# soedinglab/spacedust

Hardware: AMD Instinct MI355X
Metric: clustersearch throughput (genome-pairs/s; SW GCUPS alongside) (higher is better)
Workload: dtype int16

## Files before the change

spacedust_amd/csrc/hip/sd_sw.hip:

```cpp
#include "sd_common.h"
#include <unistd.h>


#include <algorithm>
#include <cmath>
#include <cstring>
#include <memory>
#include <omp.h>
#include <numeric>

#include "../host/sd_host.h"
#include "sd_sw_pk.h"

namespace {

using sdpk::SwTask;

template <int RT>
__global__ void __launch_bounds__(64)
sw_score_kernel(const SwTask *__restrict__ tasks, uint32_t nTasks, const uint8_t *__restrict__ qRes,
                const int8_t *__restrict__ qBias, const uint8_t *__restrict__ tRes, const int8_t *__restrict__ mat,
                int go, int ge, int32_t *__restrict__ out, uint2 *__restrict__ boundary,
                const uint32_t *__restrict__ order ,
                const int8_t *__restrict__ qProf ) {
// ... 613 lines not shown
            x = jj - x;
            ok = ok && x >= 0 && x < width_d;
            bool same = false;
            if (ok) {
                const int byte = dirs[(size_t) 16 * ii + (x >> 1)];
                const int code = (x & 1) ? (byte >> 4) : (byte & 15);
                ok = (code & 12) == 0;
                same = sq[ii] == st[jj];
            }
            const uint32_t okMask = (uint32_t) (__ballot(ok) >> sh);
            const uint32_t sameMask = (uint32_t) (__ballot(same) >> sh);
            const int run = okMask == 0xFFFFFFFFu ? 32 : __builtin_ctz(~okMask);
            const uint32_t runMask = run == 32 ? 0xFFFFFFFFu : ((1u << run) - 1u);
            if (l < run) o[-1 - l] = 'M';
            ids += __builtin_popcount(sameMask & runMask);
            i -= run;
            j -= run;
            o -= run;
            len += run;
        }
        if (going && (i > 0 || j > 0)) {
            if (i < 0 || j < 0) bad = true;
            int x = i - band;
            x = x > 0 ? x : 0;
            x = j - x;
            if (x < 0 || x >= width_d) bad = true;
            if (!bad) {
                const int byte = dirs[(size_t) 16 * i + (x >> 1)];
                const int code = (x & 1) ? (byte >> 4) : (byte & 15);
                int dcode;
                const int dE = (code & 1) ? 3 : 2, dF = (code & 2) ? 5 : 4;
                if (state == 0) dcode = dE;
                else if (state == 1) dcode = dF;
                else dcode = (code & 4) ? dE : ((code & 8) ? dF : 1);
                char c;
                switch (dcode) {
                    case 1: ids += (sq[i] == st[j]); --i; --j; state = 2; c = 'M'; break;
                    case 2: --i; state = 0; c = 'I'; break;
                    case 3: --i; state = 2; c = 'I'; break;
                    case 4: --j; state = 1; c = 'D'; break;
                    default: --j; state = 2; c = 'D'; break;
                }
                --o;
                if (l == 0) *o = c;
                len++;
            }
        }
        going = going && !bad && (i > 0 || j > 0);
    }
    if (!have || !reached || l != 0) return;
    if (bad || i != 0 || j != 0) {
        res[2 * id] = -1;
        return;
    }
    ids += (sq[0] == st[0]);
    *--o = 'M';
    len++;
    res[2 * id] = len;
    res[2 * id + 1] = ids;
}

template <int RT, int LW, bool MULTI, bool WIDE, bool SHARED>
void launchScorePk(sd_ctx *ctx, const SwTask *dTasks, const uint32_t *dOrder, uint32_t n, const sd_seqset *q,
                   const sd_seqset *t, const int8_t *dMat, int go, int ge, int32_t *dOut, uint2 *dBound) {
    if (n == 0) return;
    constexpr uint32_t perWave = 2 * (64 / LW);
    dim3 grid((n + perWave - 1) / perWave), block(64);
    static const unsigned ldsPad = getenv("SD_SW_LDS_PAD") ? (unsigned) atoi(getenv("SD_SW_LDS_PAD")) : 0u;
    hipLaunchKernelGGL((sdpk::sw_score_pk_kernel<RT, LW, MULTI, WIDE, SHARED>), grid, block, ldsPad, ctx->stream, dTasks, n, q->dRes, q->dBias,
                       t->dRes, dMat, go, ge, dOut, dBound, dOrder, (const int8_t *) q->dProf);
}

template <int RT, int LW, int SHARED, int WAVES = 1>
void launchScorePkAligned(sd_ctx *ctx, const SwTask *dTasks, const uint32_t *dOrder, uint32_t n, const sd_seqset *q, const sd_seqset *t,
                          const int8_t *dMat, int go, int ge, int32_t *dOut) {
    if (n == 0) return;
    constexpr uint32_t perWg = 2 * (64 / LW) * WAVES;
    dim3 grid((n + perWg - 1) / perWg), block(64 * WAVES);
    static const unsigned ldsPad = getenv("SD_SW_LDS_PAD") ? (unsigned) atoi(getenv("SD_SW_LDS_PAD")) : 0u;
    hipLaunchKernelGGL((sdpk::sw_score_pk_aligned_kernel<RT, LW, SHARED, WAVES>), grid, block, ldsPad, ctx->stream, dTasks, n, q->dRes, q->dBias, t->dRes,
                       dMat, go, ge, dOut, dOrder, (const int8_t *) q->dProf);
}

inline uint32_t sdSwChain() {
    const char *e = getenv("SD_SW_CHAIN");
    return e ? (uint32_t) std::min(64, std::max(0, atoi(e))) : 0u;
}
template <int RT>
void launchScorePkChain(sd_ctx *ctx, const SwTask *dTasks, const uint32_t *dOrder, uint32_t n, const sd_seqset *q, const sd_seqset *t,
                        const int8_t *dMat, int go, int ge, int32_t *dOut) {
    if (n == 0) return;
    const uint32_t nQuads = (n + 3) / 4, chainLen = sdSwChain();
    dim3 grid((nQuads + chainLen - 1) / chainLen), block(64);
    static const unsigned ldsPad = getenv("SD_SW_LDS_PAD") ? (unsigned) atoi(getenv("SD_SW_LDS_PAD")) : 0u;
    hipLaunchKernelGGL((sdpk::sw_score_pk_chain_kernel<RT>), grid, block, ldsPad, ctx->stream, dTasks, n, q->dRes, q->dBias, t->dRes, dMat, go, ge,
                       dOut, dOrder, (const int8_t *) q->dProf, chainLen);
}

int rtClass(int n) {
    if (n <= 128) return 4;
    if (n <= 256) return 8;
    if (n <= 512) return 16;
    return 32;
}

template <int RT>
void launchScore(sd_ctx *ctx, const SwTask *dTasks, uint32_t n, const sd_seqset *q, const sd_seqset *t,
                 const int8_t *dMat, int go, int ge, int32_t *dOut, uint2 *dBound) {
    if (n == 0) return;
    dim3 grid((n + 1) / 2), block(64);
    hipLaunchKernelGGL(sw_score_kernel<RT>, grid, block, 0, ctx->stream, dTasks, n, q->dRes, q->dBias, t->dRes, dMat,
                       go, ge, dOut, dBound, (const uint32_t *) nullptr, (const int8_t *) q->dProf);
}

template <int RT>
void launchScoreIdx(sd_ctx *ctx, const SwTask *dTasks, const uint32_t *dOrder, uint32_t n, const sd_seqset *q,
                    const sd_seqset *t, const int8_t *dMat, int go, int ge, int32_t *dOut, uint2 *dBound) {
    if (n == 0) return;
    dim3 grid((n + 1) / 2), block(64);
    hipLaunchKernelGGL(sw_score_kernel<RT>, grid, block, 0, ctx->stream, dTasks, n, q->dRes, q->dBias, t->dRes, dMat,
                       go, ge, dOut, dBound, dOrder, (const int8_t *) q->dProf);
}

int runScoreTasks(sd_ctx *ctx, std::vector<SwTask> &tasks, const sd_seqset *q, const sd_seqset *t, const int8_t *dMat,
                  int go, int ge, std::vector<int32_t> &hOut, uint32_t nSlots, uint64_t *cells, const char *tag = "a") {
    hOut.assign((size_t) nSlots * 3, 0);
    if (tasks.empty()) return SD_OK;
    HostScope hsAll(ctx, "score.total");
    const size_t n = tasks.size();
    constexpr int NB = 4 * 1024;
    auto keyOf = [](const SwTask &t) {
        const int c = rtClass(t.n);
        const int ci = c == 4 ? 0 : (c == 8 ? 1 : (c == 16 ? 2 : 3));
        return (uint32_t) ci * 1024u + (uint32_t) (1023 - std::min(t.tL >> 4, 1023));
    };
    SwTask *sorted = nullptr;
    SD_HIP(ctx, pinGet(ctx, (std::string("sw.tasks.") + tag).c_str(), n, &sorted));
    uint64_t boundTotal = 0, cellSum = 0;
    size_t classBegin[5] = {0, 0, 0, 0, 0};
    {
        int T = 1;
#pragma omp parallel
        {
#pragma omp single
            T = omp_get_num_threads();
        }
        T = std::max(1, std::min(T, 64));
        std::vector<uint32_t> hist((size_t) T * NB, 0);
#pragma omp parallel num_threads(T) reduction(+ : cellSum)
        {
            const int th = omp_get_thread_num();
            const size_t lo = n * th / T, hi = n * (th + 1) / T;
            uint32_t *hh = &hist[(size_t) th * NB];
            for (size_t i = lo; i < hi; i++) {
                hh[keyOf(tasks[i])]++;
                cellSum += (uint64_t) tasks[i].n * (uint64_t) tasks[i].tL;
            }
        }
        uint64_t run = 0;
        for (int bkt = 0; bkt < NB; bkt++) {
            if ((bkt & 1023) == 0) classBegin[bkt >> 10] = run;
            for (int th = 0; th < T; th++) {
                const uint32_t c = hist[(size_t) th * NB + bkt];
                hist[(size_t) th * NB + bkt] = (uint32_t) run;
                run += c;
            }
        }
        classBegin[4] = run;
#pragma omp parallel num_threads(T)
        {
            const int th = omp_get_thread_num();
            const size_t lo = n * th / T, hi = n * (th + 1) / T;
            uint32_t *hh = &hist[(size_t) th * NB];
            for (size_t i = lo; i < hi; i++) sorted[hh[keyOf(tasks[i])]++] = tasks[i];
        }
    }
    *cells += cellSum;
    for (size_t i = classBegin[3]; i < classBegin[4]; i++) {
        if (sorted[i].n > 1024) {
            sorted[i].boundOff = boundTotal;
            boundTotal += (uint64_t) sorted[i].tL;
        }
    }
    SwTask *dTasks = nullptr;
    int32_t *dOut = nullptr;
    uint2 *dBound = nullptr;
    int32_t *hPin = nullptr;
    SD_HIP(ctx, wsGet(ctx, "sw.tasks", n, &dTasks));
    SD_HIP(ctx, wsGet(ctx, "sw.out", (size_t) nSlots * 3, &dOut));
    SD_HIP(ctx, wsGet(ctx, "sw.bound", std::max<uint64_t>(boundTotal, 1), &dBound));
    SD_HIP(ctx, pinGet(ctx, "sw.hout", (size_t) nSlots * 3, &hPin));
    SD_HIP(ctx, hipMemcpyAsync(dTasks, sorted, n * sizeof(SwTask), hipMemcpyHostToDevice, ctx->stream));
    SD_HIP(ctx, hipMemsetAsync(dOut, 0, (size_t) nSlots * 3 * sizeof(int32_t), ctx->stream));
    static const int classes[4] = {4, 8, 16, 32};
    for (int ci = 0; ci < 4; ci++) {
        const size_t begin = classBegin[ci], end = classBegin[ci + 1];
        if (end == begin) continue;
        const uint32_t cnt = (uint32_t) (end - begin);
        {
            ProfScope ps(ctx, "sw_score");
            switch (classes[ci]) {
                case 4: launchScore<4>(ctx, dTasks + begin, cnt, q, t, dMat, go, ge, dOut, dBound); break;
                case 8: launchScore<8>(ctx, dTasks + begin, cnt, q, t, dMat, go, ge, dOut, dBound); break;
                case 16: launchScore<16>(ctx, dTasks + begin, cnt, q, t, dMat, go, ge, dOut, dBound); break;
                default: launchScore<32>(ctx, dTasks + begin, cnt, q, t, dMat, go, ge, dOut, dBound); break;
            }
        }
        SD_HIP(ctx, hipGetLastError());
    }
    SD_HIP(ctx, hipMemcpyAsync(hPin, dOut, (size_t) nSlots * 3 * sizeof(int32_t), hipMemcpyDeviceToHost, ctx->stream));
    SD_HIP(ctx, sdStreamSync(ctx));
    memcpy(hOut.data(), hPin, (size_t) nSlots * 3 * sizeof(int32_t));
    return SD_OK;
}


constexpr uint32_t N_NARROW_CLASSES = 24;
constexpr uint32_t FIRST_NARROW_MULTI = 21;
constexpr uint32_t N_PK_CLASSES = 14;
constexpr uint32_t FIRST_MULTI_PK = 11;
constexpr uint32_t FIRST_WIDE_CLASS = N_NARROW_CLASSES;
constexpr uint32_t FIRST_INT32_CLASS = FIRST_WIDE_CLASS + N_PK_CLASSES;
constexpr uint32_t N_SCORE_CLASSES = FIRST_INT32_CLASS + 4;
static_assert(N_SCORE_CLASSES < 63, "class boundaries are found by one 64-lane wavefront; six class bits in the pair key");
enum ScoreKernel { SCORE_PK = 0, SCORE_PK_WIDE = 1, SCORE_INT32 = 2 };
constexpr uint32_t KEY_INVALID = N_SCORE_CLASSES * 1024u;
__host__ __device__ __forceinline__ bool scoreClassIsMulti(uint32_t ci) {
    return (ci >= FIRST_NARROW_MULTI && ci < FIRST_WIDE_CLASS) || (ci >= FIRST_WIDE_CLASS + FIRST_MULTI_PK && ci < FIRST_INT32_CLASS);
}
__device__ __forceinline__ uint32_t scoreKey(int n, int tL, int kernel, int wideRowLimit = 800) {
    int ci;
    if (kernel == SCORE_PK_WIDE && min(n, tL) > wideRowLimit) kernel = SCORE_INT32;
    if (kernel == SCORE_INT32 || tL > 65535) {
        ci = FIRST_INT32_CLASS + (n <= 128 ? 0 : (n <= 256 ? 1 : (n <= 512 ? 2 : 3)));
    } else if (kernel == SCORE_PK_WIDE) {
        if (n <= 192) ci = n <= 128 ? 0 : 1;
        else if (n <= 384) ci = 2 + (n - 193) / 32;
        else if (n <= 768) ci = n <= 512 ? 8 : (n <= 640 ? 9 : 10);
        else ci = min((int) FIRST_MULTI_PK + (n + 511) / 512 - 2, 13);
        ci += FIRST_WIDE_CLASS;
    } else {
        if (n <= 128) ci = 0;
        else if (n <= 768) ci = (n + 31) / 32 - 4;
        else ci = min((int) FIRST_NARROW_MULTI + (n + 511) / 512 - 2, (int) FIRST_WIDE_CLASS - 1);
    }
    return (uint32_t) ci * 1024u + (uint32_t) (1023 - min(tL >> 4, 1023));
}

struct DevGateParams {
    int go, ge, matMin, swMode, covMode, wideRowLimit;
    float covThr;
    double evalThr;
    double lambda, K, aI, bI, alphaI, betaI, aJ, bJ, alphaJ, betaJ, sigma, tau, viThr, vjThr, cThr, dbResidues;
};

__device__ double devEvalue(const DevGateParams &e, double y_, double qLen) {
    const double m_ = e.dbResidues, n_ = qLen;
    const double const_val = 0.3989422804014327;
    double tmp = e.aI * y_ + e.bI;
    double m_li_y = m_ - tmp;
    double vi_y = fmax(e.viThr, e.alphaI * y_ + e.betaI);
    double sqrt_vi_y = sqrt(vi_y);
    double m_F = sqrt_vi_y == 0.0 ? 1e100 : m_li_y / sqrt_vi_y;
    double P_m_F = 0.5 * erfc(-sqrt(0.5) * m_F);
    double E_m_F = -const_val * exp(-0.5 * m_F * m_F);
    double p1 = m_li_y * P_m_F - sqrt_vi_y * E_m_F;
    tmp = e.aJ * y_ + e.bJ;
    double n_lj_y = n_ - tmp;
    double vj_y = fmax(e.vjThr, e.alphaJ * y_ + e.betaJ);
    double sqrt_vj_y = sqrt(vj_y);
    double n_F = sqrt_vj_y == 0.0 ? 1e100 : n_lj_y / sqrt_vj_y;
    double P_n_F = 0.5 * erfc(-sqrt(0.5) * n_F);
    double E_n_F = -const_val * exp(-0.5 * n_F * n_F);
    double p2 = n_lj_y * P_n_F - sqrt_vj_y * E_n_F;
    double c_y = fmax(e.cThr, e.sigma * y_ + e.tau);
    double area = p1 * p2 + c_y * (P_m_F * P_n_F);
    return e.K * exp(-e.lambda * y_) * area;
}

__device__ __forceinline__ float devCov(unsigned int startPos, unsigned int endPos, unsigned int len) {
    return (min(len, max(startPos, endPos)) - min(startPos, endPos) + 1) / (float) len;
}
__device__ __forceinline__ bool devHasCoverage(float covThr, int covMode, float qCov, float tCov) {
    switch (covMode) {
        case 0: return (qCov >= covThr) && (tCov >= covThr);
        case 2: return qCov >= covThr;
        case 1: return tCov >= covThr;
        default: return true;
    }
}

__global__ void __launch_bounds__(256)
k_pre_word(uint32_t nPairs, const uint32_t *__restrict__ pairQ, const uint32_t *__restrict__ pairT, const uint16_t *__restrict__ pairDiag,
           const uint32_t *__restrict__ fwdKeys, const uint64_t *__restrict__ qOff, const uint64_t *__restrict__ tOff,
           const uint8_t *__restrict__ qRes, const int8_t *__restrict__ qBias, const uint8_t *__restrict__ tRes, const int8_t *__restrict__ mat,
           const int8_t *__restrict__ qProf, const int32_t *__restrict__ minBias, int matMin, uint8_t *__restrict__ preWord,
           uint32_t *__restrict__ pass1Keys) {
    __shared__ int8_t smat[441];
    for (int x = threadIdx.x; x < 441; x += blockDim.x) smat[x] = mat[x];
    __syncthreads();
    const uint32_t i = blockIdx.x * blockDim.x + threadIdx.x;
    if (i >= nPairs) return;
    uint8_t pw = 0;
    const uint32_t key = fwdKeys[i];
    if (key != KEY_INVALID) {
        const uint64_t qo = qOff[pairQ[i]], to = tOff[pairT[i]];
        const int qL = (int) (qOff[pairQ[i] + 1] - qo), tL = (int) (tOff[pairT[i] + 1] - to);
        if (qL < 32768 && tL < 32768 && pairDiag[i] != 0x8000) {
            const int d = (int) (int16_t) pairDiag[i];
            int q0 = d >= 0 ? d : 0, t0 = d >= 0 ? 0 : -d;
            const int n = min(qL - q0, tL - t0);
            const int need = 255 - (abs(matMin) + abs(minBias[pairQ[i]]));
            int run = 0, best = 0;
            for (int x = 0; x < n && best < need; x++) {
                const int qr = qRes[qo + q0 + x], tr = tRes[to + t0 + x];
                run += qProf ? (int) qProf[(qo + q0 + x) * 21 + tr] : (int) smat[tr * 21 + qr] + (int) qBias[qo + q0 + x];
                run = run < 0 ? 0 : run;
                best = run > best ? run : best;
            }
            pw = best >= need ? 1 : 0;
        }
    }
    preWord[i] = pw;
    pass1Keys[i] = pw ? KEY_INVALID : key;
}

__global__ void __launch_bounds__(256)
// ... 464 lines not shown
    order2[2 * w] = vals[p];
    const bool mate = p + 1 < n && (keyS[p + 1] >> 9) == (keyS[p] >> 9);
    order2[2 * w + 1] = mate ? vals[p + 1] : PAIR_NONE;
}
__global__ void k_pair_bounds(const uint32_t *__restrict__ keyS, uint32_t n, const uint64_t *__restrict__ pairIdx,
                              uint32_t *__restrict__ b, int nb) {
    const int c = threadIdx.x;
    if (c >= nb) return;
    const uint32_t want = (uint32_t) c << 26;
    uint32_t lo = 0, hi = n;
    while (lo < hi) {
        const uint32_t mid = (lo + hi) >> 1;
        if (keyS[mid] < want) lo = mid + 1;
        else hi = mid;
    }
    b[c] = (uint32_t) pairIdx[lo];
}

int devRunScore(sd_ctx *ctx, uint32_t nPairs, const uint32_t *dKeys, const uint32_t *dVals, uint32_t *dKeysSorted,
                uint32_t *dOrder, uint32_t *dBounds, SwTask *dTasks, uint64_t *dScanA, uint64_t *dScanB,
                const sd_seqset *q, const sd_seqset *t, const int8_t *dMat, int go, int ge, int32_t *dOut,
                uint32_t *nValid, const uint32_t *dPairQ ) {
    const unsigned grid = (nPairs + 255) / 256;
    int rc = SD_OK;
    uint32_t *dOrder2 = nullptr, *dPairBounds = nullptr;
    if (dPairQ) {
        uint32_t *dKey2 = nullptr, *dVals2 = nullptr, *dHead = nullptr, *dRunStart = nullptr;
        uint64_t *dPairIdx = nullptr;
        uint8_t *dLeader = nullptr;
        SD_HIP(ctx, wsGet(ctx, "sp.key2", (size_t) nPairs, &dKey2));
        SD_HIP(ctx, wsGet(ctx, "sp.vals2", (size_t) nPairs, &dVals2));
        SD_HIP(ctx, wsGet(ctx, "sp.head", (size_t) nPairs, &dHead));
        SD_HIP(ctx, wsGet(ctx, "sp.runstart", (size_t) nPairs, &dRunStart));
        SD_HIP(ctx, wsGet(ctx, "sp.leader", (size_t) nPairs + 1, &dLeader));
        SD_HIP(ctx, wsGet(ctx, "sp.pairidx", (size_t) nPairs + 1, &dPairIdx));
        const int padPairs = sdSwQuads() ? 2 * sdSwWaves() : 0;
        const size_t order2Cap = (size_t) 2 * (size_t) std::max(padPairs, 2) * nPairs + 8;
        SD_HIP(ctx, wsGet(ctx, "sp.order2", order2Cap, &dOrder2));
        SD_HIP(ctx, hipMemsetAsync(dOrder2, 0xFF, order2Cap * sizeof(uint32_t), ctx->stream));
        SD_HIP(ctx, wsGet(ctx, "sp.bounds", 64, &dPairBounds));
        hipLaunchKernelGGL(k_pair_keys, dim3(grid), dim3(256), 0, ctx->stream, nPairs, dKeys, dPairQ, dKey2);
        rc = devSortPairs(ctx, dKey2, dKeysSorted, dVals, dVals2, nPairs, 32);
        if (rc != SD_OK) return rc;
        dOrder = dVals2;
        hipLaunchKernelGGL(k_pair_heads, dim3(grid), dim3(256), 0, ctx->stream, nPairs, dKeysSorted, dHead);
        rc = devInclusiveMax(ctx, dHead, dRunStart, nPairs);
        if (rc != SD_OK) return rc;
        hipLaunchKernelGGL(k_pair_leaders, dim3((nPairs + 256) / 256), dim3(256), 0, ctx->stream, nPairs, dKeysSorted, dRunStart, dLeader,
                           padPairs);
        rc = devExclusiveScan(ctx, (const uint8_t *) dLeader, dPairIdx, (size_t) nPairs + 1);
        if (rc != SD_OK) return rc;
        hipLaunchKernelGGL(k_pair_emit, dim3(grid), dim3(256), 0, ctx->stream, nPairs, dKeysSorted, dVals2, dRunStart, dPairIdx, dOrder2);
        hipLaunchKernelGGL(k_pair_bounds, dim3(1), dim3(64), 0, ctx->stream, dKeysSorted, nPairs, dPairIdx, dPairBounds,
                           (int) FIRST_INT32_CLASS + 1);
        hipLaunchKernelGGL(k_bounds, dim3(1), dim3(64), 0, ctx->stream, dKeysSorted, nPairs, 1u << 26, dBounds, (int) N_SCORE_CLASSES + 1);
    } else {
        rc = devSortPairs(ctx, dKeys, dKeysSorted, dVals, dOrder, nPairs, 16);
        if (rc != SD_OK) return rc;
        hipLaunchKernelGGL(k_bounds, dim3(1), dim3(64), 0, ctx->stream, dKeysSorted, nPairs, 1024u, dBounds, (int) N_SCORE_CLASSES + 1);
    }
    hipLaunchKernelGGL(k_bound_need, dim3(grid), dim3(256), 0, ctx->stream, nPairs, dTasks, dKeys, dScanA);
    SD_HIP(ctx, hipMemsetAsync(dScanA + nPairs, 0, sizeof(uint64_t), ctx->stream));
    rc = devExclusiveScan(ctx, dScanA, dScanB, (size_t) nPairs + 1);
    if (rc != SD_OK) return rc;
    hipLaunchKernelGGL(k_bound_apply, dim3(grid), dim3(256), 0, ctx->stream, nPairs, dTasks, dScanB);
    uint32_t hb[N_SCORE_CLASSES + 1], hpb[FIRST_INT32_CLASS + 1];
    uint64_t boundTotal = 0;
    if (dPairQ) SD_HIP(ctx, sdD2H(ctx, hpb, dPairBounds, sizeof(hpb)));
    SD_HIP(ctx, sdD2H(ctx, hb, dBounds, sizeof(hb)));
    SD_HIP(ctx, sdD2H(ctx, &boundTotal, dScanB + nPairs, sizeof(uint64_t)));
    SD_HIP(ctx, sdStreamSync(ctx));
    *nValid = hb[N_SCORE_CLASSES];
    uint2 *dBound = nullptr;
    SD_HIP(ctx, wsGet(ctx, "sw.bound", std::max<uint64_t>(boundTotal, 1), &dBound));
    for (uint32_t ci = 0; ci < N_SCORE_CLASSES; ci++) {
        const uint32_t begin = hb[ci], cnt = hb[ci + 1] - hb[ci];
        if (cnt == 0) continue;
        static const char *const pkNames[N_PK_CLASSES] = {"rt4x32", "rt6x32", "rt7x32", "rt8x32", "rt9x32", "rt10x32", "rt11x32", "rt12x32",
                                                          "rt8x64", "rt10x64", "rt12x64", "rt8x64s2", "rt8x64s3", "rt8x64sN"};
        static const char *const i32Names[4] = {"sw_score.rt4", "sw_score.rt8", "sw_score.rt16", "sw_score.rt32"};
        static const bool long32 = !(getenv("SD_SW_LONG32") && atoi(getenv("SD_SW_LONG32")) == 0);
        static const bool useAligned = !(getenv("SD_SW_ALIGNED") && atoi(getenv("SD_SW_ALIGNED")) == 0);
        const bool shared = dPairQ != nullptr && ci < FIRST_INT32_CLASS;
        const int alignedRT = (ci >= 1 && ci < FIRST_NARROW_MULTI) ? (int) ci + 4 : 0;
        const bool aligned = alignedRT > 0 && useAligned && (alignedRT <= 12 || (shared && long32));
        int generalIdx = 0;
        if (ci >= FIRST_NARROW_MULTI && ci < FIRST_WIDE_CLASS) generalIdx = (int) FIRST_MULTI_PK + (int) (ci - FIRST_NARROW_MULTI);
        else if (alignedRT) generalIdx = alignedRT <= 6 ? 1 : (alignedRT <= 12 ? alignedRT - 5 : (alignedRT <= 16 ? 8 : (alignedRT <= 20 ? 9 : 10)));
        char name[48];
        if (aligned) snprintf(name, sizeof(name), "sw_score_pk.a_seg%d", alignedRT);
        else if (ci < FIRST_WIDE_CLASS) snprintf(name, sizeof(name), "sw_score_pk.%s", pkNames[generalIdx]);
        else if (ci < FIRST_INT32_CLASS) snprintf(name, sizeof(name), "sw_score_pk.w_%s", pkNames[ci - FIRST_WIDE_CLASS]);
        else snprintf(name, sizeof(name), "%s", i32Names[ci - FIRST_INT32_CLASS]);
        ProfScope ps(ctx, name);
        const uint32_t *ord = dOrder + begin;
        uint32_t nOrd = cnt;
        if (shared) {
            ord = dOrder2 + 2 * (size_t) hpb[ci];
            nOrd = 2 * (hpb[ci + 1] - hpb[ci]);
        }
#define SD_PK(RT, LW, MULTI, WIDE)                                                                                          \
    do {                                                                                                                   \
        if (shared) launchScorePk<RT, LW, MULTI, WIDE, true>(ctx, dTasks, ord, nOrd, q, t, dMat, go, ge, dOut, dBound);     \
        else launchScorePk<RT, LW, MULTI, WIDE, false>(ctx, dTasks, ord, nOrd, q, t, dMat, go, ge, dOut, dBound);           \
    } while (0)
#define SD_PKA(RT)                                                                                               \
    case RT:                                                                                                     \
        if (shared && quads && sdSwWaves() == 2) launchScorePkAligned<RT, 32, 2, 2>(ctx, dTasks, ord, nOrd, q, t, dMat, go, ge, dOut);  \
        else if (shared && quads && sdSwChain() > 1) launchScorePkChain<RT>(ctx, dTasks, ord, nOrd, q, t, dMat, go, ge, dOut);  \
        else if (shared && quads) launchScorePkAligned<RT, 32, 2>(ctx, dTasks, ord, nOrd, q, t, dMat, go, ge, dOut);  \
        else if (shared) launchScorePkAligned<RT, 32, 1>(ctx, dTasks, ord, nOrd, q, t, dMat, go, ge, dOut);      \
        else launchScorePkAligned<RT, 32, 0>(ctx, dTasks, ord, nOrd, q, t, dMat, go, ge, dOut);                  \
        break;
#define SD_PKA16(SEG)                                                                                            \
    case SEG: launchScorePkAligned<2 * SEG, 16, 1>(ctx, dTasks, ord, nOrd, q, t, dMat, go, ge, dOut); break;
#define SD_PK_CLASS(WIDE, IDX)                                                \
        switch (IDX) {                                                        \
            case 0: SD_PK(4, 32, false, WIDE); break;                         \
            case 1: SD_PK(6, 32, false, WIDE); break;                         \
            case 2: SD_PK(7, 32, false, WIDE); break;                         \
            case 3: SD_PK(8, 32, false, WIDE); break;                         \
            case 4: SD_PK(9, 32, false, WIDE); break;                         \
            case 5: SD_PK(10, 32, false, WIDE); break;                        \
            case 6: SD_PK(11, 32, false, WIDE); break;                        \
            case 7: SD_PK(12, 32, false, WIDE); break;                        \
            case 8: SD_PK(8, 64, false, WIDE); break;                         \
            case 9: SD_PK(10, 64, false, WIDE); break;                        \
            case 10: SD_PK(12, 64, false, WIDE); break;                       \
            default: SD_PK(8, 64, true, WIDE); break;                         \
        }
        static const int lw16Max = getenv("SD_SW_LW16") ? atoi(getenv("SD_SW_LW16")) : (sdSwQuads() ? 0 : 8);
        const bool quads = sdSwQuads();
        if (aligned && shared && alignedRT <= lw16Max) {
            switch (alignedRT) {
                SD_PKA16(5) SD_PKA16(6) SD_PKA16(7) SD_PKA16(8) SD_PKA16(9) SD_PKA16(10) SD_PKA16(11) SD_PKA16(12)
                default: break;
            }
        } else if (aligned) {
            switch (alignedRT) {
                SD_PKA(5) SD_PKA(6) SD_PKA(7) SD_PKA(8) SD_PKA(9) SD_PKA(10) SD_PKA(11) SD_PKA(12) SD_PKA(13) SD_PKA(14)
                SD_PKA(15) SD_PKA(16) SD_PKA(17) SD_PKA(18) SD_PKA(19) SD_PKA(20) SD_PKA(21) SD_PKA(22) SD_PKA(23) SD_PKA(24)
                default: break;
            }
        } else if (ci < FIRST_WIDE_CLASS) {
            SD_PK_CLASS(false, generalIdx)
        } else if (ci < FIRST_INT32_CLASS) {
            SD_PK_CLASS(true, (int) (ci - FIRST_WIDE_CLASS))
        } else {
            switch (ci - FIRST_INT32_CLASS) {
                case 0: launchScoreIdx<4>(ctx, dTasks, ord, cnt, q, t, dMat, go, ge, dOut, dBound); break;
                case 1: launchScoreIdx<8>(ctx, dTasks, ord, cnt, q, t, dMat, go, ge, dOut, dBound); break;
                case 2: launchScoreIdx<16>(ctx, dTasks, ord, cnt, q, t, dMat, go, ge, dOut, dBound); break;
                default: launchScoreIdx<32>(ctx, dTasks, ord, cnt, q, t, dMat, go, ge, dOut, dBound); break;
            }
        }
#undef SD_PKA
#undef SD_PKA16
#undef SD_PK_CLASS
#undef SD_PK
    }
    SD_HIP(ctx, hipGetLastError());
    return SD_OK;
}

__global__ void __launch_bounds__(256)
k_cells(uint32_t nPairs, const SwTask *__restrict__ tasks, const uint32_t *__restrict__ keys, unsigned long long *__restrict__ acc) {
    const uint32_t i = blockIdx.x * blockDim.x + threadIdx.x;
    unsigned long long c = 0;
    if (i < nPairs && keys[i] != KEY_INVALID) c = (unsigned long long) tasks[i].n * (unsigned long long) tasks[i].tL;
#pragma unroll
    for (int off = 32; off >= 1; off >>= 1) c += __shfl_xor(c, off, 64);
    if ((threadIdx.x & 63) == 0 && c) atomicAdd(acc, c);
}

}

int sdFail(sd_ctx *ctx, int code, const char *fmt, ...) {
    char buf[1024];
    va_list ap;
    va_start(ap, fmt);
    vsnprintf(buf, sizeof(buf), fmt, ap);
    va_end(ap);
    if (ctx) ctx->lastError = buf;
    else fprintf(stderr, "spacedust_gpu: %s\n", buf);
    return code;
}

extern "C" {

int sd_ctx_create(int device, sd_ctx **out) { return sd_ctx_create_prio(device, 0, out); }

int sd_ctx_create_prio(int device, int priority, sd_ctx **out) { return sd_ctx_create_masked(device, priority, 0, out); }

int sd_ctx_create_masked(int device, int priority, int reserveCUs, sd_ctx **out) {
    if (out == nullptr) return SD_EINVAL;
    *out = nullptr;
    int count = 0;
    hipError_t e = hipGetDeviceCount(&count);
    if (e != hipSuccess || count <= 0) {
        fprintf(stderr, "spacedust_gpu: no HIP device visible (%s); this library has no CPU fallback\n",
                e != hipSuccess ? hipGetErrorString(e) : "device count 0");
        return SD_ENODEVICE;
    }
    if (device < 0 || device >= count) return SD_EINVAL;
    if (hipSetDevice(device) != hipSuccess) return SD_ENODEVICE;
    sd_ctx *c = new sd_ctx();
    c->device = device;
    int least = 0, greatest = 0;
    (void) hipDeviceGetStreamPriorityRange(&least, &greatest);
    const int prio = priority < 0 ? greatest : (priority > 0 ? least : (least + greatest) / 2);
    hipError_t se = hipSuccess;
    (void) hipGetDeviceProperties(&c->prop, device);
    const int nCU = c->prop.multiProcessorCount;
    if (reserveCUs > 0 && nCU > 0 && reserveCUs < nCU) {
        std::vector<uint32_t> mask((size_t) (nCU + 31) / 32, 0u);
        for (int b = 0; b < nCU - reserveCUs; b++) mask[(size_t) b / 32] |= 1u << (b % 32);
        se = hipExtStreamCreateWithCUMask(&c->stream, (uint32_t) mask.size(), mask.data());
    } else {
        se = hipStreamCreateWithPriority(&c->stream, hipStreamNonBlocking, prio);
    }
    if (se != hipSuccess) {
        delete c;
        return SD_EHIP;
    }
    const char *syncMode = getenv("SD_SYNC");
    const bool spin = syncMode && strcmp(syncMode, "spin") == 0;
    (void) hipEventCreate(&c->evStart);
    (void) hipEventCreate(&c->evStop);
    if (!spin) (void) hipEventCreateWithFlags(&c->evSync, hipEventDisableTiming);
    (void) hipGetDeviceProperties(&c->prop, device);
    *out = c;
    return SD_OK;
}

void sd_ctx_destroy(sd_ctx *ctx) {
    if (!ctx) return;
    (void) hipSetDevice(ctx->device);
    if (ctx->evStart) (void) hipEventDestroy(ctx->evStart);
    if (ctx->evStop) (void) hipEventDestroy(ctx->evStop);
    if (ctx->evSync) (void) hipEventDestroy(ctx->evSync);
// ... 1105 lines not shown
```

spacedust_amd/csrc/hip/sd_sw_pk.h:

```cpp
#ifndef SD_SW_PK_H
#define SD_SW_PK_H

#include <hip/hip_runtime.h>
#include <cstdint>

namespace sdpk {

struct SwTask {
    uint64_t qOff;
    uint64_t tOff;
    int32_t n;
    int32_t tL;
    int32_t qStep;
    int32_t tStep;
    int32_t segLen;
    uint32_t slot;
    uint64_t boundOff;
};

typedef short s16x2 __attribute__((ext_vector_type(2)));
typedef unsigned short u16x2 __attribute__((ext_vector_type(2)));

__device__ __forceinline__ uint32_t pkMax(uint32_t a, uint32_t b) {
    return __builtin_bit_cast(uint32_t, __builtin_elementwise_max(__builtin_bit_cast(s16x2, a), __builtin_bit_cast(s16x2, b)));
// ... 530 lines not shown
            const uint32_t aA = addWord0(baseA, Tn), aB = addWord1(baseB, Tn);
#pragma unroll
            for (int w = 0; w < WORDS; w++) {
                pan[w] = ldsWord(aA, w);
                pbn[w] = ldsWord(aB, w);
            }
        }
        uint32_t inG, inFf;
        if (LW == 16) {
            inG = dppMove<0x111, true>(0, outG);
            inFf = dppMove<0x111, true>(0, outFf);
        } else {
            inG = dppShr1(outG);
            inFf = dppShr1(outFf);
            inG = writeLane<32>(0, inG);
            inFf = writeLane<32>(0, inFf);
        }
        uint32_t h[RTP];
#pragma unroll
        for (int w = 0; w < WORDS; w++) {
            const uint32_t d0 = (w == 0) ? prevInG : H[4 * w - 1];
            addProfile4(pac[w], pbc[w], d0, H[4 * w], H[4 * w + 1], H[4 * w + 2], h[4 * w], h[4 * w + 1], h[4 * w + 2], h[4 * w + 3]);
        }
        prevInG = inG;
        uint32_t Fl = 0, Ff = inFf, cm = 0;
#pragma unroll
        for (int r = 0; r < RT; r++) {
            uint32_t hpre = pkMax(h[r], E[r]);
            if (r % SEG != 0) hpre = pkMax(hpre, Fl);
            const uint32_t g = pkMax(hpre, Ff);
            const uint32_t open = pkSubSat(hpre, goP);
            E[r] = pkMax(pkSubSat(E[r], geP), open);
            if (r % SEG == 0) Fl = open;
            else if ((r + 1) % SEG != 0) Fl = pkMax(pkSubSat(Fl, geP), open);
            Ff = pkMax(pkSubSat(Ff, geP), open);
            H[r] = g;
            const uint32_t code = pkRowCode(g, 31 - r);
            cm = r == 0 ? code : pkMax(cm, code);
        }
        outG = H[RT - 1];
        outFf = Ff;
        const uint32_t t = bestcm | 0x001F001Fu;
        const uint32_t m = pkAshr15(pkSub(t, cm));
        const uint32_t kk = (uint32_t) k | ((uint32_t) k << 16);
        bestcm = bfiAsm(m, cm, bestcm);
        bestcol = bfiAsm(m, kk, bestcol);
    };
    uint32_t T2, pa2[WORDS], pb2[WORDS];
#pragma unroll 1
    for (int k = 0; k < steps; k += 2) {
        columnStep(k, T, pa, pb, T2, pa2, pb2);
        columnStep(k + 1, T2, pa2, pb2, T, pa, pb);
    }
    unsigned long long keyA = 0, keyB = 0;
    {
        const uint32_t vA = (bestcm & 0xFFFFu) >> 5, vB = bestcm >> 21;
        const uint32_t rowA = (uint32_t) (q0 + 31 - (int) (bestcm & 31u)), rowB = (uint32_t) (q0 + 31 - (int) ((bestcm >> 16) & 31u));
        const uint32_t colA = (bestcol & 0xFFFFu) - (uint32_t) l, colB = (bestcol >> 16) - (uint32_t) l;
        if (vA > 0) keyA = ((unsigned long long) vA << 40) | ((unsigned long long) (0xFFFFFu - colA) << 20) | (unsigned long long) (0xFFFFFu - rowA);
        if (vB > 0) keyB = ((unsigned long long) vB << 40) | ((unsigned long long) (0xFFFFFu - colB) << 20) | (unsigned long long) (0xFFFFFu - rowB);
    }
#pragma unroll
    for (int off = LW / 2; off >= 1; off >>= 1) {
        const unsigned long long oa = __shfl_xor(keyA, off, LW), ob = __shfl_xor(keyB, off, LW);
        keyA = oa > keyA ? oa : keyA;
        keyB = ob > keyB ? ob : keyB;
    }
    if (l == 0) {
        if (haveA) {
            const int v = (int) (keyA >> 40);
            out[3 * A.slot + 0] = v;
            out[3 * A.slot + 1] = v == 0 ? -1 : 0xFFFFF - (int) ((keyA >> 20) & 0xFFFFF);
            out[3 * A.slot + 2] = v == 0 ? A.n - 1 : 0xFFFFF - (int) (keyA & 0xFFFFF);
        }
        if (haveB) {
            const int v = (int) (keyB >> 40);
            out[3 * B.slot + 0] = v;
            out[3 * B.slot + 1] = v == 0 ? -1 : 0xFFFFF - (int) ((keyB >> 20) & 0xFFFFF);
            out[3 * B.slot + 2] = v == 0 ? B.n - 1 : 0xFFFFF - (int) (keyB & 0xFFFFF);
        }
    }
}


template <int RT>
__global__ void __launch_bounds__(64)
sw_score_pk_chain_kernel(const SwTask *__restrict__ tasks, uint32_t nTasks, const uint8_t *__restrict__ qRes,
                         const int8_t *__restrict__ qBias, const uint8_t *__restrict__ tRes, const int8_t *__restrict__ mat,
                         int go, int ge, int32_t *__restrict__ out, const uint32_t *__restrict__ order,
                         const int8_t *__restrict__ qProf, uint32_t chainLen) {
    constexpr int LW = 32;
    constexpr int WORDS = (RT + 3) / 4;
    constexpr int RTP = 4 * WORDS;
    constexpr int PSTRIDE = LW * WORDS;
    constexpr uint32_t ROWB = PSTRIDE * 4;
    static_assert(22 * ROWB < 65536, "row offsets travel in 16 bits");
    __shared__ uint32_t prof[22][PSTRIDE];
    __shared__ int8_t smat[441];
    for (int i = threadIdx.x; i < 441; i += 64) smat[i] = mat[i];
    __syncthreads();
    const int lane = threadIdx.x;
    const int grp = lane >> 5, l = lane & 31;
    const int q0 = l * RT;
    const uint32_t goP = (uint32_t) go | ((uint32_t) go << 16), geP = (uint32_t) ge | ((uint32_t) ge << 16);
    constexpr uint32_t NEUT = (uint32_t) PK_NEUTRAL * ROWB;
    typedef __attribute__((address_space(3))) uint32_t lds_u32;
    const uint32_t base = (uint32_t) (size_t) (lds_u32 *) (&prof[0][0] + l * WORDS);
    auto ldsWord = [](uint32_t addr, int w) -> uint32_t { return *((const lds_u32 *) (size_t) addr + w); };

    const uint32_t nQuads = (nTasks + 3) / 4;
    uint32_t qd = blockIdx.x * chainLen;
    const uint32_t qdEnd = min(qd + chainLen, nQuads);
    auto loadQuad = [&](uint32_t quad, SwTask (&tk)[4]) {
#pragma unroll
        for (int x = 0; x < 4; x++) {
            const uint32_t id = quad * 4 + x;
            const uint32_t tid = id < nTasks ? (order ? order[id] : id) : 0xFFFFFFFFu;
            if (tid != 0xFFFFFFFFu) {
                tk[x] = tasks[tid];
            } else {
                tk[x].n = 0; tk[x].tL = 0; tk[x].qOff = 0; tk[x].tOff = 0; tk[x].qStep = 1; tk[x].tStep = 1; tk[x].segLen = 1;
                tk[x].slot = 0; tk[x].boundOff = 0;
            }
        }
    };
    bool firstChain = true;
    while (qd < qdEnd) {
        SwTask tk[4];
        loadQuad(qd, tk);
        if (tk[0].n <= 0) {
            qd++;
            continue;
        }
        if (!firstChain) __syncthreads();
        firstChain = false;
        const SwTask Q = tk[0];
        {
            uint32_t *pw = &prof[0][0] + l * WORDS;
#pragma unroll
            for (int w = 0; w < WORDS; w++) {
                int res[4], cb[4];
                int64_t pidx[4];
                bool valid[4];
#pragma unroll
                for (int b = 0; b < 4; b++) {
                    const int qi = q0 + 4 * w + b;
                    valid[b] = (4 * w + b < RT) && qi < Q.n;
                    res[b] = 20;
                    cb[b] = 0;
                    pidx[b] = 0;
                    if (valid[b]) {
                        const int64_t idx = (int64_t) Q.qOff + (int64_t) qi * Q.qStep;
                        res[b] = qRes[idx];
                        cb[b] = qBias[idx];
                        pidx[b] = idx * 21;
                    }
                }
                if (qProf) {
                    for (int a = grp; a < 21; a += 2) {
                        uint32_t word = 0;
#pragma unroll
                        for (int b = 0; b < 4; b++) {
                            const int v = valid[b] ? (int) qProf[pidx[b] + a] : -64;
                            word |= (uint32_t) (uint8_t) (int8_t) v << (8 * b);
                        }
                        pw[a * PSTRIDE + w] = word;
// ... 206 lines not shown
```

Baseline: 2772.

## Route wide-score pairs through a new aligned word-profile kernel with fine class buckets

Wide-score pairs used to fall into a few coarse PK classes. They are now bucketed into the same fine 32-row classes as narrow pairs. Aligned wide classes dispatch to a new sw_score_pk_word_kernel, which splits each segment over two or four lanes (LW 32 or 64). It packs a byte-wise query profile into LDS and tracks the best cell per row with bit-field selects. The intent is to cut padding waste and register pressure for wide tasks, at the cost of many more template instantiations, extra LDS use and a changed class layout.

```diff
diff --git a/spacedust_amd/csrc/hip/sd_sw.hip b/spacedust_amd/csrc/hip/sd_sw.hip
--- a/spacedust_amd/csrc/hip/sd_sw.hip
+++ b/spacedust_amd/csrc/hip/sd_sw.hip
@@ -719,6 +719,17 @@
                        dMat, go, ge, dOut, dOrder, (const int8_t *) q->dProf);
 }
 
+template <int RT, int LW, int SHARE>
+void launchScorePkWord(sd_ctx *ctx, const SwTask *dTasks, const uint32_t *dOrder, uint32_t n, const sd_seqset *q, const sd_seqset *t,
+                       const int8_t *dMat, int go, int ge, int32_t *dOut) {
+    if (n == 0) return;
+    constexpr uint32_t perWave = 2 * (64 / LW);
+    dim3 grid((n + perWave - 1) / perWave), block(64);
+    static const unsigned ldsPad = getenv("SD_SW_LDS_PAD") ? (unsigned) atoi(getenv("SD_SW_LDS_PAD")) : 0u;
+    hipLaunchKernelGGL((sdpk::sw_score_pk_word_kernel<RT, LW, SHARE>), grid, block, ldsPad, ctx->stream, dTasks, n, q->dRes, q->dBias, t->dRes,
+                       dMat, go, ge, dOut, dOrder, (const int8_t *) q->dProf);
+}
+
 inline uint32_t sdSwChain() {
     const char *e = getenv("SD_SW_CHAIN");
     return e ? (uint32_t) std::min(64, std::max(0, atoi(e))) : 0u;
@@ -857,29 +868,24 @@
 constexpr uint32_t N_PK_CLASSES = 14;
 constexpr uint32_t FIRST_MULTI_PK = 11;
 constexpr uint32_t FIRST_WIDE_CLASS = N_NARROW_CLASSES;
-constexpr uint32_t FIRST_INT32_CLASS = FIRST_WIDE_CLASS + N_PK_CLASSES;
+constexpr uint32_t FIRST_INT32_CLASS = FIRST_WIDE_CLASS + N_NARROW_CLASSES;
 constexpr uint32_t N_SCORE_CLASSES = FIRST_INT32_CLASS + 4;
 static_assert(N_SCORE_CLASSES < 63, "class boundaries are found by one 64-lane wavefront; six class bits in the pair key");
 enum ScoreKernel { SCORE_PK = 0, SCORE_PK_WIDE = 1, SCORE_INT32 = 2 };
 constexpr uint32_t KEY_INVALID = N_SCORE_CLASSES * 1024u;
 __host__ __device__ __forceinline__ bool scoreClassIsMulti(uint32_t ci) {
-    return (ci >= FIRST_NARROW_MULTI && ci < FIRST_WIDE_CLASS) || (ci >= FIRST_WIDE_CLASS + FIRST_MULTI_PK && ci < FIRST_INT32_CLASS);
+    return (ci >= FIRST_NARROW_MULTI && ci < FIRST_WIDE_CLASS) || (ci >= FIRST_WIDE_CLASS + FIRST_NARROW_MULTI && ci < FIRST_INT32_CLASS);
 }
 __device__ __forceinline__ uint32_t scoreKey(int n, int tL, int kernel, int wideRowLimit = 800) {
     int ci;
     if (kernel == SCORE_PK_WIDE && min(n, tL) > wideRowLimit) kernel = SCORE_INT32;
     if (kernel == SCORE_INT32 || tL > 65535) {
         ci = FIRST_INT32_CLASS + (n <= 128 ? 0 : (n <= 256 ? 1 : (n <= 512 ? 2 : 3)));
-    } else if (kernel == SCORE_PK_WIDE) {
-        if (n <= 192) ci = n <= 128 ? 0 : 1;
-        else if (n <= 384) ci = 2 + (n - 193) / 32;
-        else if (n <= 768) ci = n <= 512 ? 8 : (n <= 640 ? 9 : 10);
-        else ci = min((int) FIRST_MULTI_PK + (n + 511) / 512 - 2, 13);
-        ci += FIRST_WIDE_CLASS;
     } else {
         if (n <= 128) ci = 0;
         else if (n <= 768) ci = (n + 31) / 32 - 4;
         else ci = min((int) FIRST_NARROW_MULTI + (n + 511) / 512 - 2, (int) FIRST_WIDE_CLASS - 1);
+        if (kernel == SCORE_PK_WIDE) ci += FIRST_WIDE_CLASS;
     }
     return (uint32_t) ci * 1024u + (uint32_t) (1023 - min(tL >> 4, 1023));
 }
@@ -1510,15 +1516,16 @@
         static const bool long32 = !(getenv("SD_SW_LONG32") && atoi(getenv("SD_SW_LONG32")) == 0);
         static const bool useAligned = !(getenv("SD_SW_ALIGNED") && atoi(getenv("SD_SW_ALIGNED")) == 0);
         const bool shared = dPairQ != nullptr && ci < FIRST_INT32_CLASS;
-        const int alignedRT = (ci >= 1 && ci < FIRST_NARROW_MULTI) ? (int) ci + 4 : 0;
-        const bool aligned = alignedRT > 0 && useAligned && (alignedRT <= 12 || (shared && long32));
+        const bool wide = ci >= FIRST_WIDE_CLASS && ci < FIRST_INT32_CLASS;
+        const uint32_t rc = wide ? ci - FIRST_WIDE_CLASS : ci;
+        const int alignedRT = (rc >= 1 && rc < FIRST_NARROW_MULTI) ? (int) rc + 4 : 0;
+        const bool aligned = alignedRT > 0 && useAligned && (alignedRT <= 12 || (long32 && (shared || wide)));
         int generalIdx = 0;
-        if (ci >= FIRST_NARROW_MULTI && ci < FIRST_WIDE_CLASS) generalIdx = (int) FIRST_MULTI_PK + (int) (ci - FIRST_NARROW_MULTI);
+        if (rc >= FIRST_NARROW_MULTI && rc < FIRST_WIDE_CLASS) generalIdx = (int) FIRST_MULTI_PK + (int) (rc - FIRST_NARROW_MULTI);
         else if (alignedRT) generalIdx = alignedRT <= 6 ? 1 : (alignedRT <= 12 ? alignedRT - 5 : (alignedRT <= 16 ? 8 : (alignedRT <= 20 ? 9 : 10)));
         char name[48];
-        if (aligned) snprintf(name, sizeof(name), "sw_score_pk.a_seg%d", alignedRT);
-        else if (ci < FIRST_WIDE_CLASS) snprintf(name, sizeof(name), "sw_score_pk.%s", pkNames[generalIdx]);
-        else if (ci < FIRST_INT32_CLASS) snprintf(name, sizeof(name), "sw_score_pk.w_%s", pkNames[ci - FIRST_WIDE_CLASS]);
+        if (aligned) snprintf(name, sizeof(name), "sw_score_pk.%sa_seg%d", wide ? "w_" : "", alignedRT);
+        else if (ci < FIRST_INT32_CLASS) snprintf(name, sizeof(name), "sw_score_pk.%s%s", wide ? "w_" : "", pkNames[generalIdx]);
         else snprintf(name, sizeof(name), "%s", i32Names[ci - FIRST_INT32_CLASS]);
         ProfScope ps(ctx, name);
         const uint32_t *ord = dOrder + begin;
@@ -1542,6 +1549,13 @@
         break;
 #define SD_PKA16(SEG)                                                                                            \
     case SEG: launchScorePkAligned<2 * SEG, 16, 1>(ctx, dTasks, ord, nOrd, q, t, dMat, go, ge, dOut); break;
+#define SD_PKW(RT)                                                                                               \
+    case RT:                                                                                                     \
+        if (shared && quads) launchScorePkWord<RT, 32, 2>(ctx, dTasks, ord, nOrd, q, t, dMat, go, ge, dOut);     \
+        else if (shared) launchScorePkWord<RT, 32, 1>(ctx, dTasks, ord, nOrd, q, t, dMat, go, ge, dOut);         \
+        else if (RT <= 12) launchScorePkWord<(RT <= 12 ? RT : 12), 32, 0>(ctx, dTasks, ord, nOrd, q, t, dMat, go, ge, dOut);  \
+        else launchScorePkWord<(RT > 12 ? (RT + 1) / 2 : 7), 64, 0>(ctx, dTasks, ord, nOrd, q, t, dMat, go, ge, dOut);\
+        break;
 #define SD_PK_CLASS(WIDE, IDX)                                                \
         switch (IDX) {                                                        \
             case 0: SD_PK(4, 32, false, WIDE); break;                         \
@@ -1559,7 +1573,13 @@
         }
         static const int lw16Max = getenv("SD_SW_LW16") ? atoi(getenv("SD_SW_LW16")) : (sdSwQuads() ? 0 : 8);
         const bool quads = sdSwQuads();
-        if (aligned && shared && alignedRT <= lw16Max) {
+        if (aligned && wide) {
+            switch (alignedRT) {
+                SD_PKW(5) SD_PKW(6) SD_PKW(7) SD_PKW(8) SD_PKW(9) SD_PKW(10) SD_PKW(11) SD_PKW(12) SD_PKW(13) SD_PKW(14)
+                SD_PKW(15) SD_PKW(16) SD_PKW(17) SD_PKW(18) SD_PKW(19) SD_PKW(20) SD_PKW(21) SD_PKW(22) SD_PKW(23) SD_PKW(24)
+                default: break;
+            }
+        } else if (aligned && shared && alignedRT <= lw16Max) {
             switch (alignedRT) {
                 SD_PKA16(5) SD_PKA16(6) SD_PKA16(7) SD_PKA16(8) SD_PKA16(9) SD_PKA16(10) SD_PKA16(11) SD_PKA16(12)
                 default: break;
@@ -1573,7 +1593,7 @@
         } else if (ci < FIRST_WIDE_CLASS) {
             SD_PK_CLASS(false, generalIdx)
         } else if (ci < FIRST_INT32_CLASS) {
-            SD_PK_CLASS(true, (int) (ci - FIRST_WIDE_CLASS))
+            SD_PK_CLASS(true, generalIdx)
         } else {
             switch (ci - FIRST_INT32_CLASS) {
                 case 0: launchScoreIdx<4>(ctx, dTasks, ord, cnt, q, t, dMat, go, ge, dOut, dBound); break;
@@ -1584,6 +1604,7 @@
         }
 #undef SD_PKA
 #undef SD_PKA16
+#undef SD_PKW
 #undef SD_PK_CLASS
 #undef SD_PK
     }
diff --git a/spacedust_amd/csrc/hip/sd_sw_pk.h b/spacedust_amd/csrc/hip/sd_sw_pk.h
--- a/spacedust_amd/csrc/hip/sd_sw_pk.h
+++ b/spacedust_amd/csrc/hip/sd_sw_pk.h
@@ -636,6 +636,255 @@
     }
 }
 
+template <int RT, int LW, int SHARE>
+__global__ void __launch_bounds__(64)
+sw_score_pk_word_kernel(const SwTask *__restrict__ tasks, uint32_t nTasks, const uint8_t *__restrict__ qRes,
+                        const int8_t *__restrict__ qBias, const uint8_t *__restrict__ tRes, const int8_t *__restrict__ mat,
+                        int go, int ge, int32_t *__restrict__ out, const uint32_t *__restrict__ order,
+                        const int8_t *__restrict__ qProf) {
+    static_assert(LW == 32 || LW == 64, "two or four lanes per segment of the word kernel");
+    constexpr int LPS = LW / 16;
+    static_assert(RT >= LPS, "the last lane of a segment holds at least one real row");
+    constexpr int WORDS = (RT + 3) / 4;
+    constexpr int RTP = 4 * WORDS;
+    constexpr int PSTRIDE = LW * WORDS;
+    constexpr int NGRP = 64 / LW;
+    constexpr int NT = 2 * NGRP;
+    constexpr uint32_t ROWB = PSTRIDE * 4;
+    static_assert(22 * ROWB < 65536, "row offsets travel in 16 bits");
+    constexpr bool SHARED = SHARE != 0;
+    __shared__ uint32_t prof[SHARE == 2 ? 1 : (SHARE == 1 ? NGRP : NT)][22][PSTRIDE];
+    __shared__ int8_t smat[441];
+    for (int i = threadIdx.x; i < 441; i += 64) smat[i] = mat[i];
+    __syncthreads();
+    const int lane = threadIdx.x;
+    const int grp = lane / LW, l = lane % LW;
+    const int seg = l / LPS, j = l % LPS;
+    SwTask tk[NT];
+#pragma unroll
+    for (int x = 0; x < NT; x++) {
+        const uint32_t id = blockIdx.x * NT + x;
+        const uint32_t tid = id < nTasks ? (order ? order[id] : id) : 0xFFFFFFFFu;
+        if (tid != 0xFFFFFFFFu) {
+            tk[x] = tasks[tid];
+        } else {
+            tk[x].n = 0; tk[x].tL = 0; tk[x].qOff = 0; tk[x].tOff = 0; tk[x].qStep = 1; tk[x].tStep = 1; tk[x].segLen = 1;
+            tk[x].slot = 0; tk[x].boundOff = 0;
+        }
+    }
+    SwTask A = tk[0], B = tk[1];
+    if (NGRP == 2 && grp) {
+        A = tk[NT - 2];
+        B = tk[NT - 1];
+    }
+    const bool haveA = A.n > 0, haveB = B.n > 0;
+    if (SHARED && !haveB) {
+        B = A;
+        B.tL = 0;
+    }
+    int maxN = 0, maxTL = 0;
+#pragma unroll
+    for (int x = 0; x < NT; x++) {
+        maxN = max(maxN, tk[x].n);
+        maxTL = max(maxTL, tk[x].tL);
+    }
+    const int steps = (maxN > 0 && maxTL > 0) ? maxTL + LW - 1 : 0;
+    const uint32_t goP = (uint32_t) go | ((uint32_t) go << 16), geP = (uint32_t) ge | ((uint32_t) ge << 16);
+    const int q0A = seg * A.segLen + j * RT, q0B = seg * B.segLen + j * RT;
+    const int rowsA = j + 1 < LPS ? RT : A.segLen - (LPS - 1) * RT, rowsB = j + 1 < LPS ? RT : B.segLen - (LPS - 1) * RT;
+#pragma unroll
+    for (int x = 0; x < (SHARED ? 1 : 2); x++) {
+        const SwTask &T = SHARE == 2 ? tk[0] : (x ? B : A);
+        const int q0 = SHARE == 2 ? seg * T.segLen + j * RT : (x ? q0B : q0A);
+        const int rows = SHARE == 2 ? (j + 1 < LPS ? RT : T.segLen - (LPS - 1) * RT) : (x ? rowsB : rowsA);
+        uint32_t *pw = &prof[SHARE == 2 ? 0 : (SHARE == 1 ? grp : 2 * grp + x)][0][0] + l * WORDS;
+#pragma unroll
+        for (int w = 0; w < WORDS; w++) {
+            int res[4], cb[4];
+            int64_t pidx[4];
+            bool valid[4];
+#pragma unroll
+            for (int b = 0; b < 4; b++) {
+                const int qi = q0 + 4 * w + b;
+                valid[b] = (4 * w + b < rows) && qi < T.n;
+                res[b] = 20;
+                cb[b] = 0;
+                pidx[b] = 0;
+                if (valid[b]) {
+                    const int64_t idx = (int64_t) T.qOff + (int64_t) qi * T.qStep;
+                    res[b] = qRes[idx];
+                    cb[b] = qBias[idx];
+                    pidx[b] = idx * 21;
+                }
+            }
+            const int aFirst = SHARE == 2 ? grp : 0, aStep = SHARE == 2 ? NGRP : 1;
+            if (qProf) {
+                for (int a = aFirst; a < 21; a += aStep) {
+                    uint32_t word = 0;
+#pragma unroll
+                    for (int b = 0; b < 4; b++) {
+                        const int v = valid[b] ? (int) qProf[pidx[b] + a] : -64;
+                        word |= (uint32_t) (uint8_t) (int8_t) v << (8 * b);
+                    }
+                    pw[a * PSTRIDE + w] = word;
+                }
+            } else {
+                for (int a = aFirst; a < 21; a += aStep) {
+                    uint32_t word = 0;
+#pragma unroll
+                    for (int b = 0; b < 4; b++) {
+                        const int v = valid[b] ? (int) smat[a * 21 + res[b]] + cb[b] : -64;
+                        word |= (uint32_t) (uint8_t) (int8_t) v << (8 * b);
+                    }
+                    pw[a * PSTRIDE + w] = word;
+                }
+            }
+            pw[PK_NEUTRAL * PSTRIDE + w] = 0xC0C0C0C0u;
+        }
+    }
+    __syncthreads();
+    const uint32_t flKeep = j != 0 ? 0xFFFFFFFFu : 0u;
+    uint32_t padSel[LPS];
+#pragma unroll
+    for (int p = 0; p < LPS; p++)
+        padSel[p] = (j + 1 == LPS) ? ((RT - rowsA == p ? 0x0000FFFFu : 0u) | (RT - rowsB == p ? 0xFFFF0000u : 0u)) : 0u;
+    typedef __attribute__((address_space(3))) uint32_t lds_u32;
+    const uint32_t baseA = (uint32_t) (size_t) (lds_u32 *) (&prof[SHARE == 2 ? 0 : (SHARE == 1 ? grp : 2 * grp)][0][0] + l * WORDS);
+    const uint32_t baseB = SHARED ? baseA : (uint32_t) (size_t) (lds_u32 *) (&prof[2 * grp + 1][0][0] + l * WORDS);
+    auto ldsWord = [](uint32_t addr, int w) -> uint32_t { return *((const lds_u32 *) (size_t) addr + w); };
+
+    uint32_t H[RTP], E[RTP], bestH[RT];
+#pragma unroll
+    for (int r = 0; r < RTP; r++) {
+        H[r] = 0;
+        E[r] = 0;
+    }
+#pragma unroll
+    for (int r = 0; r < RT; r++) bestH[r] = 0;
+    uint32_t outG = 0, outFf = 0, outFl = 0, prevInG = 0;
+    uint32_t bestv = 0, bestcol = 0;
+    constexpr uint32_t NEUT = (uint32_t) PK_NEUTRAL * ROWB;
+    auto loadChunk = [&](int c0) -> uint32_t {
+        const int col = c0 + l;
+        uint32_t a = PK_NEUTRAL, b = PK_NEUTRAL;
+        if (col < A.tL) a = tRes[(int64_t) A.tOff + (int64_t) col * A.tStep];
+        if (col < B.tL) b = tRes[(int64_t) B.tOff + (int64_t) col * B.tStep];
+        return (a * ROWB) | ((b * ROWB) << 16);
+    };
+    uint32_t chunk = loadChunk(0);
+    uint32_t chunkNext = loadChunk(LW);
+    uint32_t T = NEUT | (NEUT << 16);
+    T = writeLane<0>(readLane(chunk, 0), T);
+    if (NGRP == 2) T = writeLane<32>(readLane(chunk, 32), T);
+    uint32_t pa[WORDS], pb[WORDS];
+    {
+        const uint32_t aA = addWord0(baseA, T), aB = addWord1(baseB, T);
+#pragma unroll
+        for (int w = 0; w < WORDS; w++) {
+            pa[w] = ldsWord(aA, w);
+            pb[w] = ldsWord(aB, w);
+        }
+    }
+    auto columnStep = [&](const int k, const uint32_t &Tc, const uint32_t (&pac)[WORDS], const uint32_t (&pbc)[WORDS], uint32_t &Tn,
+                          uint32_t (&pan)[WORDS], uint32_t (&pbn)[WORDS]) {
+        const int i1 = (k + 1) & (LW - 1);
+        if (i1 == 0) {
+            chunk = chunkNext;
+            chunkNext = loadChunk(k + 1 + LW);
+        }
+        Tn = dppShr1(Tc);
+        Tn = writeLane<0>(readLane(chunk, i1), Tn);
+        if (NGRP == 2) Tn = writeLane<32>(readLane(chunk, 32 + i1), Tn);
+        {
+            const uint32_t aA = addWord0(baseA, Tn), aB = addWord1(baseB, Tn);
+#pragma unroll
+            for (int w = 0; w < WORDS; w++) {
+                pan[w] = ldsWord(aA, w);
+                pbn[w] = ldsWord(aB, w);
+            }
+        }
+        uint32_t inG = dppShr1(outG), inFf = dppShr1(outFf);
+        const uint32_t inFl = dppShr1(outFl) & flKeep;
+        if (NGRP == 2) {
+            inG = writeLane<32>(0, inG);
+            inFf = writeLane<32>(0, inFf);
+        }
+        uint32_t h[RTP];
+#pragma unroll
+        for (int w = 0; w < WORDS; w++) {
+            const uint32_t d0 = (w == 0) ? prevInG : H[4 * w - 1];
+            addProfile4(pac[w], pbc[w], d0, H[4 * w], H[4 * w + 1], H[4 * w + 2], h[4 * w], h[4 * w + 1], h[4 * w + 2], h[4 * w + 3]);
+        }
+        prevInG = inG;
+        uint32_t Fl = inFl, Ff = inFf, cm = 0, FfAt[LPS];
+#pragma unroll
+        for (int r = 0; r < RT; r++) {
+            const uint32_t hpre = pkMax(pkMax(h[r], E[r]), Fl);
+            const uint32_t g = pkMax(hpre, Ff);
+            const uint32_t open = pkSubSat(hpre, goP);
+            E[r] = pkMax(pkSubSat(E[r], geP), open);
+            Fl = pkMax(pkSubSat(Fl, geP), open);
+            Ff = pkMax(pkSubSat(Ff, geP), open);
+            H[r] = g;
+            if (r >= RT - LPS) FfAt[RT - 1 - r] = Ff;
+            cm = r == 0 ? g : pkMax(cm, g);
+        }
+        outFl = Fl;
+        outG = H[RT - 1];
+        outFf = FfAt[0];
+#pragma unroll
+        for (int p = 1; p < LPS; p++) {
+            outG = bfiAsm(padSel[p], H[RT - 1 - p], outG);
+            outFf = bfiAsm(padSel[p], FfAt[p], outFf);
+        }
+        const uint32_t m = pkAshr15(pkSub(bestv, cm));
+        const uint32_t kk = (uint32_t) k | ((uint32_t) k << 16);
+        bestv = pkMax(bestv, cm);
+        bestcol = bfiAsm(m, kk, bestcol);
+#pragma unroll
+        for (int r = 0; r < RT; r++) bestH[r] = bfiAsm(m, H[r], bestH[r]);
+    };
+    uint32_t T2, pa2[WORDS], pb2[WORDS];
+#pragma unroll 1
+    for (int k = 0; k < steps; k += 2) {
+        columnStep(k, T, pa, pb, T2, pa2, pb2);
+        columnStep(k + 1, T2, pa2, pb2, T, pa, pb);
+    }
+    unsigned long long keyA = 0, keyB = 0;
+    {
+        const uint32_t vA = bestv & 0xFFFFu, vB = bestv >> 16;
+        int rA = 0, rB = 0;
+#pragma unroll
+        for (int r = RT - 1; r >= 0; r--) {
+            if ((bestH[r] & 0xFFFFu) == vA) rA = r;
+            if ((bestH[r] >> 16) == vB) rB = r;
+        }
+        const uint32_t rowA = (uint32_t) (q0A + rA), rowB = (uint32_t) (q0B + rB);
+        const uint32_t colA = ((bestcol & 0xFFFFu) - (uint32_t) l) & 0xFFFFu, colB = ((bestcol >> 16) - (uint32_t) l) & 0xFFFFu;
+        if (vA > 0) keyA = ((unsigned long long) vA << 40) | ((unsigned long long) (0xFFFFFu - colA) << 20) | (unsigned long long) (0xFFFFFu - rowA);
+        if (vB > 0) keyB = ((unsigned long long) vB << 40) | ((unsigned long long) (0xFFFFFu - colB) << 20) | (unsigned long long) (0xFFFFFu - rowB);
+    }
+#pragma unroll
+    for (int off = LW / 2; off >= 1; off >>= 1) {
+        const unsigned long long oa = __shfl_xor(keyA, off, LW), ob = __shfl_xor(keyB, off, LW);
+        keyA = oa > keyA ? oa : keyA;
+        keyB = ob > keyB ? ob : keyB;
+    }
+    if (l == 0) {
+        if (haveA) {
+            const int v = (int) (keyA >> 40);
+            out[3 * A.slot + 0] = v;
+            out[3 * A.slot + 1] = v == 0 ? -1 : 0xFFFFF - (int) ((keyA >> 20) & 0xFFFFF);
+            out[3 * A.slot + 2] = v == 0 ? A.n - 1 : 0xFFFFF - (int) (keyA & 0xFFFFF);
+        }
+        if (haveB) {
+            const int v = (int) (keyB >> 40);
+            out[3 * B.slot + 0] = v;
+            out[3 * B.slot + 1] = v == 0 ? -1 : 0xFFFFF - (int) ((keyB >> 20) & 0xFFFFF);
+            out[3 * B.slot + 2] = v == 0 ? B.n - 1 : 0xFFFFF - (int) (keyB & 0xFFFFF);
+        }
+    }
+}
 
 template <int RT>
 __global__ void __launch_bounds__(64)
```

After: 2839, median of 6. 2.4% higher.
